# architector1324/micro-raytracer

Measured on AMD Instinct MI355X. Metric: Msamples/sec (res x spp), higher is better.
Workload: dtype f32

## Files before the change

### micro_raytracer_amd/csrc/mrt_math.h

```cpp
#pragma once

#include <stdint.h>

#if defined(__HIPCC__) || defined(__HIP__)
#define MRT_HD __host__ __device__ inline __attribute__((always_inline))
#define MRT_HD_NOINLINE __host__ __device__
#else
#define MRT_HD inline __attribute__((always_inline))
#define MRT_HD_NOINLINE
#endif

namespace mrt {

typedef uint32_t u32;
typedef int32_t i32;

MRT_HD u32 f2u(float f) { return __builtin_bit_cast(u32, f); }
MRT_HD float u2f(u32 u) { return __builtin_bit_cast(float, u); }
MRT_HD float fabs_(float x) { return __builtin_fabsf(x); }
MRT_HD float floor_(float x) { return __builtin_floorf(x); }
MRT_HD float trunc_(float x) { return __builtin_truncf(x); }

#if defined(__HIP_DEVICE_COMPILE__) && !defined(MRT_GENERIC_IEEE)
#define MRT_FAST_IEEE 1
MRT_HD bool wave_all(bool ok) { return __builtin_amdgcn_ballot_w64(!ok) == 0ull; }
#else
MRT_HD bool wave_all(bool ok) { return ok; }
#endif
constexpr float kWinLo = 0x1p-40f, kWinHi = 0x1p+40f;
MRT_HD bool in_window(float x) { const float a = fabs_(x); return a >= kWinLo && a <= kWinHi; }
MRT_HD bool in_window_pos(float x) { return x >= kWinLo && x <= kWinHi; }

#if defined(MRT_FAST_IEEE)
MRT_HD float sqrt_core_(float x)
{
    const float s = __builtin_amdgcn_sqrtf(x);
    const float sd = u2f(f2u(s) - 1u), su = u2f(f2u(s) + 1u);
    const float vd = __builtin_fmaf(-sd, s, x), vu = __builtin_fmaf(-su, s, x);
    float r = (0.0f >= vd) ? sd : s;
    r = (0.0f < vu) ? su : r;
    return r;
}
MRT_HD float rcp_refined_(float d)
{
    const float r0 = __builtin_amdgcn_rcpf(d);
    const float e = __builtin_fmaf(-d, r0, 1.0f);
    return __builtin_fmaf(e, r0, r0);
}
MRT_HD float div_core_(float n, float d, float r)
{
    const float q0 = n * r;
    const float q1 = __builtin_fmaf(__builtin_fmaf(-d, q0, n), r, q0);
    return __builtin_fmaf(__builtin_fmaf(-d, q1, n), r, q1);
}
#endif

MRT_HD float sqrt_(float x)
{
#if defined(MRT_FAST_IEEE)
    if (wave_all(in_window_pos(x))) return sqrt_core_(x);
#endif
    return __builtin_sqrtf(x);
}
MRT_HD float recip_(float x)
{
#if defined(MRT_FAST_IEEE)
    if (wave_all(in_window(x))) return div_core_(1.0f, x, rcp_refined_(x));
#endif
    return 1.0f / x;
}
MRT_HD float div_(float a, float b)
{
#if defined(MRT_FAST_IEEE)
    if (wave_all(in_window(a) && in_window(b))) return div_core_(a, b, rcp_refined_(b));
#endif
    return a / b;
}
MRT_HD void div2_(float a0, float a1, float b, float &q0, float &q1)
{
#if defined(MRT_FAST_IEEE)
    if (wave_all(in_window(a0) && in_window(a1) && in_window(b))) {
        const float r = rcp_refined_(b);
        q0 = div_core_(a0, b, r);
        q1 = div_core_(a1, b, r);
        return;
    }
#endif
    q0 = a0 / b;
    q1 = a1 / b;
}
MRT_HD float recip_sqrt_(float m)
{
#if defined(MRT_FAST_IEEE)
    if (wave_all(in_window_pos(m))) {
        const float s = sqrt_core_(m);
        return div_core_(1.0f, s, rcp_refined_(s));
    }
#endif
    return 1.0f / __builtin_sqrtf(m);
}
MRT_HD float rcp_fast(float x)
{
#if defined(__HIP_DEVICE_COMPILE__)
    return __builtin_amdgcn_rcpf(x);
#else
    return 1.0f / x;
#endif
}
MRT_HD float fma_(float a, float b, float c) { return __builtin_fmaf(a, b, c); }
MRT_HD float fma_fast(float a, float b, float c)
{
#if defined(__HIP_DEVICE_COMPILE__)
    return __builtin_fmaf(a, b, c);
#else
    return a * b + c;
#endif
}

constexpr float kPi = 3.14159274101257324f;
constexpr float kPiO2 = 1.57079637050628662f;
constexpr float kPiO4 = 0.785398185253143311f;
constexpr float kInf = __builtin_huge_valf();

MRT_HD float qnan() { return u2f(0x7fc00000u); }

#if defined(__HIP_DEVICE_COMPILE__)
MRT_HD float fmax_(float a, float b) { return __builtin_fmaxf(a, b); }
MRT_HD float fmin_(float a, float b) { return __builtin_fminf(a, b); }
#else
MRT_HD float fmax_(float a, float b)
{
    if (a != a) return b;
    if (b != b) return a;
    if (a == b) return (f2u(a) & 0x80000000u) ? b : a;
    return a < b ? b : a;
}
MRT_HD float fmin_(float a, float b)
{
    if (a != a) return b;
    if (b != b) return a;
    if (a == b) return (f2u(a) & 0x80000000u) ? a : b;
    return b < a ? b : a;
}
#endif

MRT_HD void sincos_(float x, float &s, float &c)
{
    if (!(fabs_(x) <= 65536.0f)) { s = qnan(); c = qnan(); return; }
    const float kf = floor_(fma_(x, 0.636619746685028076f, 0.5f));
    float r = fma_(-kf, 1.5703125f, x);
    r = fma_(-kf, 4.83751296997070312e-4f, r);
    r = fma_(-kf, 7.54978995489188216e-8f, r);
    const float z = r * r;
    const float sp = fma_(fma_(fma_(-1.9515295891e-4f, z, 8.3321608736e-3f), z, -1.6666654611e-1f) * z, r, r);
    const float cp = fma_(fma_(fma_(2.443315711809948e-5f, z, -1.388731625493765e-3f), z, 4.166664568298827e-2f) * z, z,
                          fma_(-0.5f, z, 1.0f));
    const int q = (int)kf & 3;
    float ss = (q & 1) ? cp : sp;
    float cc = (q & 1) ? sp : cp;
    if (q & 2) ss = -ss;
    if ((q + 1) & 2) cc = -cc;
    s = ss;
    c = cc;
}

MRT_HD float asin_core_(float a)
{
    const float z = a * a;
    const float p = fma_(fma_(fma_(fma_(4.2163199048e-2f, z, 2.4181311049e-2f), z, 4.5470025998e-2f), z, 7.4953002686e-2f), z, 1.6666752422e-1f);
    return fma_(p * z, a, a);
}

MRT_HD float acos_(float x)
{
    const float ax = fabs_(x);
    const bool big = ax > 0.5f;
    const float s = sqrt_(0.5f * (1.0f - ax));
    const float p = asin_core_(big ? s : x);
    const float two_p = 2.0f * p;
    const float r_big = (x > 0.0f) ? two_p : kPi - two_p;
    return big ? r_big : kPiO2 - p;
}

MRT_HD float atan_pos_(float t)
{
    float y0, x;
    if (t > 2.414213562373095f) { y0 = kPiO2; x = -recip_(t); }
    else if (t > 0.4142135623730950f) { y0 = kPiO4; x = div_(t - 1.0f, t + 1.0f); }
    else { y0 = 0.0f; x = t; }
    const float z = x * x;
    const float p = fma_(fma_(fma_(8.05374449538e-2f, z, -1.38776856032e-1f), z, 1.99777106478e-1f), z, -3.33329491539e-1f);
    return y0 + fma_(p * z, x, x);
}

MRT_HD float atan2_(float y, float x)
{
    if (x != x || y != y) return qnan();
    const float ay = fabs_(y), ax = fabs_(x);
    float a;
    if (ax == 0.0f) {
        if (ay == 0.0f) return 0.0f;
        a = kPiO2;
    } else if (ay == kInf && ax == kInf) {
        a = kPiO4;
    } else {
        a = atan_pos_(div_(ay, ax));
    }
    if (x < 0.0f) a = kPi - a;
    return (y < 0.0f) ? -a : a;
}

MRT_HD float pow_(float xf, float yf)
{
    if (yf == 0.0f) return 1.0f;
    if (xf != xf || yf != yf) return qnan();
    if (xf < 0.0f) return qnan();
    if (xf == 0.0f) return (yf > 0.0f) ? 0.0f : kInf;
    if (xf == kInf) return (yf > 0.0f) ? kInf : 0.0f;
    if (xf == 1.0f) return 1.0f;
    if (yf == kInf) return (xf > 1.0f) ? kInf : 0.0f;
    if (yf == -kInf) return (xf > 1.0f) ? 0.0f : kInf;

    const double x = (double)xf;
    const uint64_t bits = __builtin_bit_cast(uint64_t, x);
    int e = (int)((bits >> 52) & 0x7ff) - 1023;
    double m = __builtin_bit_cast(double, (bits & 0x000fffffffffffffULL) | 0x3ff0000000000000ULL);
    if (m > 1.4142135623730951) { m = m * 0.5; e = e + 1; }
    const double r = (m - 1.0) / (m + 1.0);
    const double r2 = r * r;
    double p = 1.0 / 23.0;
    p = p * r2 + 1.0 / 21.0;
    p = p * r2 + 1.0 / 19.0;
    p = p * r2 + 1.0 / 17.0;
    p = p * r2 + 1.0 / 15.0;
    p = p * r2 + 1.0 / 13.0;
    p = p * r2 + 1.0 / 11.0;
    p = p * r2 + 1.0 / 9.0;
    p = p * r2 + 1.0 / 7.0;
    p = p * r2 + 1.0 / 5.0;
    p = p * r2 + 1.0 / 3.0;
    p = p * r2 + 1.0;
    const double lnm = 2.0 * r * p;
    const double log2x = (double)e + lnm * 1.4426950408889634;
    const double t = (double)yf * log2x;
    if (t >= 129.0) return kInf;
    if (t <= -151.0) return 0.0f;
    const double kf = __builtin_floor(t + 0.5);
    const double f = (t - kf) * 0.6931471805599453;
    double q = 1.0 / 6227020800.0;
    q = q * f + 1.0 / 479001600.0;
    q = q * f + 1.0 / 39916800.0;
    q = q * f + 1.0 / 3628800.0;
    q = q * f + 1.0 / 362880.0;
    q = q * f + 1.0 / 40320.0;
    q = q * f + 1.0 / 5040.0;
    q = q * f + 1.0 / 720.0;
    q = q * f + 1.0 / 120.0;
    q = q * f + 1.0 / 24.0;
    q = q * f + 1.0 / 6.0;
    q = q * f + 0.5;
// ... 39 lines not shown
```

### micro_raytracer_amd/csrc/mrt_trace.h

```cpp
#pragma once
#include "mrt_scene.h"

namespace mrt {

enum : u32 {
    F_BOX = 1u,
    F_TRI = 2u,
    F_MAPS = 4u,
    F_LIGHTS = 8u,
    F_ALL = 15u,
    F_BVH = 16u,
    F_NOSTASH = 32u,
    F_COLD = 64u,
    F_DEEP = 128u,
    F_IDENT = 256u
};
constexpr u32 plain_feat(u32 feat) { return feat & ~(u32)F_IDENT; }
MRT_HD u32 staged_words_for(const Params &P, u32 feat) { return (feat & F_DEEP) ? P.lds_words_hot : ((feat & F_COLD) ? P.lds_words_warm : P.lds_words); }
constexpr bool has_walk_area(u32 feat) { return (feat & F_TRI) && (feat & F_BOX) && (feat & F_COLD); }
#ifndef MRT_UNIFORM_TAG
#define MRT_UNIFORM_TAG 1
#endif
#ifndef MRT_T0_FROM_KEY
#define MRT_T0_FROM_KEY 1
#endif
#ifndef MRT_NZFIN_PRODUCT
#define MRT_NZFIN_PRODUCT 1
#endif
#ifndef MRT_SHADOW_QUEUE
#define MRT_SHADOW_QUEUE 0
#endif
#ifndef MRT_LEAF_QUEUE
#define MRT_LEAF_QUEUE 8u
#endif
constexpr u32 kLeafQueue = MRT_LEAF_QUEUE;

#ifndef MRT_PROBE
#define MRT_PROBE(phase)
#endif
#ifndef MRT_COUNT
#define MRT_COUNT(counter)
#endif
#ifndef MRT_PROBE_INST
#define MRT_PROBE_INST(i)
#endif
#if defined(MRT_PHASE_TIMING) && defined(__HIP_DEVICE_COMPILE__)
#define MRT_TICK(slot) do { const unsigned long long now_ = __builtin_amdgcn_s_memtime(); phase_ticks[slot] += now_ - phase_last; phase_last = now_; } while (0)
#define MRT_TICK_DECL unsigned long long phase_ticks[4] = {0ull, 0ull, 0ull, 0ull}; unsigned long long phase_last = __builtin_amdgcn_s_memtime()
#define MRT_TICK_OUT(dst) do { for (int k_ = 0; k_ < 4; ++k_) (dst)[k_] = phase_ticks[k_]; } while (0)
#else
#define MRT_TICK(slot)
#define MRT_TICK_DECL
#define MRT_TICK_OUT(dst)
#endif
#ifndef MRT_PROBE_FALLBACK
#define MRT_PROBE_FALLBACK(ro, rd, dd)
#endif
#ifndef MRT_PROBE_ROUND
#define MRT_PROBE_ROUND(steps, tris, membs)
#endif
enum : u32 { CT_TRACE = 0, CT_LIN_TEST, CT_BVH_NODE, CT_BVH_TEST, CT_MESH_CALL, CT_MESH_ROOT_HIT, CT_TBVH_NODE, CT_TBVH_TRI, CT_TBVH_TRI_HIT, CT_MEMB_BOX, CT_TRACE_ANY, CT_WALK_OVERFLOW, CT_WALK_ROUND, CT_REF_TRI, CT_REF_BOX, CT_COUNT };
enum : u32 { PH_ITER = 0, PH_REGEN, PH_SPHERE_MATH, PH_PLANE_HIT, PH_SHADE, PH_NORMAL_NONPLANE, PH_SCATTER1, PH_SCATTER2, PH_REFRACT, PH_EMIT_END, PH_LIGHTS, PH_COUNT };

constexpr float kE = 0.0001f;
constexpr float kBig = 1.0f / 0.0001f;

struct V3 { float x, y, z; };
MRT_HD V3 v3(float x, float y, float z) { V3 r; r.x = x; r.y = y; r.z = z; return r; }
MRT_HD V3 add(V3 a, V3 b) { return v3(a.x + b.x, a.y + b.y, a.z + b.z); }
MRT_HD V3 sub(V3 a, V3 b) { return v3(a.x - b.x, a.y - b.y, a.z - b.z); }
MRT_HD float dot(V3 a, V3 b) { return a.x * b.x + a.y * b.y + a.z * b.z; }
MRT_HD V3 muls(V3 a, float s) { return v3(a.x * s, a.y * s, a.z * s); }
MRT_HD V3 neg(V3 a) { return v3(-a.x, -a.y, -a.z); }
MRT_HD V3 hadam(V3 a, V3 b) { return v3(a.x * b.x, a.y * b.y, a.z * b.z); }
MRT_HD V3 cross(V3 a, V3 b) { return v3(a.y * b.z - a.z * b.y, a.z * b.x - a.x * b.z, a.x * b.y - a.y * b.x); }
MRT_HD float mag(V3 a) { return sqrt_(a.x * a.x + a.y * a.y + a.z * a.z); }
MRT_HD V3 norm(V3 a) { return muls(a, recip_sqrt_(a.x * a.x + a.y * a.y + a.z * a.z)); }
MRT_HD V3 reflect(V3 d, V3 n) { return sub(d, muls(n, 2.0f * dot(d, n))); }
MRT_HD V3 m3mul(const float *m, V3 v)
{
    return v3(m[0] * v.x + m[1] * v.y + m[2] * v.z, m[3] * v.x + m[4] * v.y + m[5] * v.z, m[6] * v.x + m[7] * v.y + m[8] * v.z);
}
MRT_HD V3 ld3(const float *F, u32 i) { return v3(F[i], F[i + 1], F[i + 2]); }
struct alignas(16) F4 { float x, y, z, w; };
MRT_HD F4 ld4(const float *F, u32 i) { return *reinterpret_cast<const F4 *>(F + i); }
MRT_HD u32 ldu(const float *F, u32 i) { return f2u(F[i]); }

MRT_HD bool nzfin(float x)
{
#if defined(__HIP_DEVICE_COMPILE__)
    return __builtin_amdgcn_classf(x, 0x198);
#else
    const float a = fabs_(x);
    return a > 0.0f && a < kInf;
#endif
}
MRT_HD bool nzfin3(V3 v) { return nzfin(v.x) && nzfin(v.y) && nzfin(v.z); }
MRT_HD bool nzfin3_product(V3 v) { return MRT_NZFIN_PRODUCT ? nzfin((v.x * v.y) * v.z) : nzfin3(v); }
MRT_HD u32 mul24(u32 a, u32 b)
{
    return (a & 0xffffffu) * (b & 0xffffffu);
}
MRT_HD void sched_fence()
{
#if defined(__HIP_DEVICE_COMPILE__)
    __builtin_amdgcn_sched_barrier(0);
#endif
}
MRT_HD u32 opaque_v(u32 x)
{
#if defined(__HIP_DEVICE_COMPILE__)
    asm volatile("" : "+v"(x));
#endif
    return x;
}
MRT_HD u32 opaque_s(u32 x)
{
#if defined(__HIP_DEVICE_COMPILE__)
    asm volatile("" : "+s"(x));
#endif
    return x;
}
MRT_HD u32 lowest_bit(u32 x) { return (u32)__builtin_ctz(x | 0x80000000u); }

MRT_HD V3 xf_full(const float *X, V3 v) { return m3mul(X + XF_R, m3mul(X + XF_L, v)); }
MRT_HD V3 xf_vec(const float *X, bool ident, V3 v)
{
    if (ident && nzfin3_product(v)) return v;
    return xf_full(X, v);
}

MRT_HD V3 recip_patched(V3 d)
{
    V3 m;
#if defined(MRT_FAST_IEEE)
    if (wave_all(in_window(d.x) && in_window(d.y) && in_window(d.z))) {
        m = v3(div_core_(1.0f, d.x, rcp_refined_(d.x)), div_core_(1.0f, d.y, rcp_refined_(d.y)), div_core_(1.0f, d.z, rcp_refined_(d.z)));
        return m;
    }
#endif
    m = v3(1.0f / d.x, 1.0f / d.y, 1.0f / d.z);
    if (fabs_(m.x) == kInf) m.x = kBig;
    if (fabs_(m.y) == kInf) m.y = kBig;
    if (fabs_(m.z) == kInf) m.z = kBig;
    return m;
}

MRT_HD bool box_isect(V3 half, V3 ro, V3 m, V3 pos, float &t0, float &t1)
{
    const V3 n = hadam(sub(ro, pos), m);
    const V3 k = hadam(half, v3(fabs_(m.x), fabs_(m.y), fabs_(m.z)));
    const V3 a = sub(neg(n), k);
    const V3 b = add(neg(n), k);
    t0 = fmax_(fmax_(a.x, a.y), a.z);
    t1 = fmin_(fmin_(b.x, b.y), b.z);
    return !(t0 > t1 || t1 < 0.0f);
}

MRT_HD bool sphere_isect(float r2, V3 oo, V3 rd, float a, float &t0, float &t1)
{
    const float b = 2.0f * dot(oo, rd);
    const float c = dot(oo, oo) - r2;
    const float disc = b * b - 4.0f * a * c;
    if (disc < 0.0f) return false;
    if (b > 1e-20f && a > 0.0f && a < 1e18f && disc >= 0.0f) return false;
    MRT_PROBE(PH_SPHERE_MATH);
    const float sq = sqrt_(disc);
    float q0, q1;
    div2_(-b - sq, -b + sq, 2.0f * a, q0, q1);
    if (q0 < 0.0f) return false;
    t0 = q0;
    t1 = q1;
    return true;
}

MRT_HD bool tri_isect(V3 vp, V3 e0, V3 e1, V3 ro, V3 rd, float &t)
{
    const V3 p = cross(rd, e1);
    const float d = dot(e0, p);
    if (d < kE && d > -kE) return false;
    const float inv_d = recip_(d);
    const V3 tv = sub(ro, vp);
    const float u = dot(tv, p) * inv_d;
    if (u < 0.0f || u > 1.0f) return false;
    const V3 q = cross(tv, e0);
    const float v = dot(rd, q) * inv_d;
    if (v < 0.0f || (u + v) > 1.0f) return false;
    const float tt = dot(e1, q) * inv_d;
    if (tt < 0.0f) return false;
    t = tt;
    return true;
}

MRT_HD bool plane_isect(V3 nn, float d, V3 ro, V3 rd, float &t)
{
    const float tt = div_(-(dot(ro, nn) + d), dot(rd, nn));
    if (tt <= 0.0f) return false;
    t = tt;
    return true;
}

MRT_HD bool in_range(float lo, float hi, float x) { return lo <= x && x < hi; }

MRT_HD V3 box_normal(V3 inv2, V3 hit, V3 pos)
{
    const V3 p = hadam(sub(hit, pos), inv2);
    const float plo = 1.0f - kE, phi = 1.0f + kE, nlo = -1.0f - kE, nhi = -1.0f + kE;
    V3 n = v3(0.0f, 0.0f, 0.0f);
    if (in_range(plo, phi, p.x)) n = v3(1.0f, 0.0f, 0.0f);
    else if (in_range(nlo, nhi, p.x)) n = v3(-1.0f, -0.0f, -0.0f);
    else if (in_range(plo, phi, p.y)) n = v3(0.0f, 1.0f, 0.0f);
    else if (in_range(nlo, nhi, p.y)) n = v3(-0.0f, -1.0f, -0.0f);
    if (in_range(plo, phi, p.z)) n = v3(0.0f, 0.0f, 1.0f);
    else if (in_range(nlo, nhi, p.z)) n = v3(-0.0f, -0.0f, -1.0f);
    return n;
}

struct UV { float x, y; };

MRT_HD UV box_uv(V3 inv2, V3 hit, V3 pos)
{
    const V3 p = hadam(sub(hit, pos), inv2);
    const float plo = 1.0f - kE, phi = 1.0f + kE, nlo = -1.0f - kE, nhi = -1.0f + kE;
    UV r;
    if (in_range(plo, phi, p.x)) { r.x = (0.5f + 0.5f * p.y) / 4.0f + 2.0f / 4.0f; r.y = div_(0.5f - 0.5f * p.z, 3.0f) + 1.0f / 3.0f; }
    else if (in_range(nlo, nhi, p.x)) { r.x = (0.5f - 0.5f * p.y) / 4.0f; r.y = div_(0.5f - 0.5f * p.z, 3.0f) + 1.0f / 3.0f; }
    else if (in_range(plo, phi, p.y)) { r.x = (0.5f - 0.5f * p.x) / 4.0f + 3.0f / 4.0f; r.y = div_(0.5f - 0.5f * p.z, 3.0f) + 1.0f / 3.0f; }
    else if (in_range(nlo, nhi, p.y)) { r.x = (0.5f + 0.5f * p.x) / 4.0f + 1.0f / 4.0f; r.y = div_(0.5f - 0.5f * p.z, 3.0f) + 1.0f / 3.0f; }
    else if (in_range(plo, phi, p.z)) { r.x = (0.5f + 0.5f * p.x) / 4.0f + 1.0f / 4.0f; r.y = div_(0.5f - 0.5f * p.y, 3.0f); }
    else if (in_range(nlo, nhi, p.z)) { r.x = (0.5f + 0.5f * p.x) / 4.0f + 1.0f / 4.0f; r.y = div_(0.5f + 0.5f * p.y, 3.0f) + 2.0f / 3.0f; }
    else { r.x = 0.0f; r.y = 0.0f; }
    return r;
}

MRT_HD float fract_(float x) { return x - trunc_(x); }

MRT_HD uint64_t to_index(float v)
{
    if (!(v > 0.0f)) return 0;
    if (v >= 2147483648.0f) return 2147483648ull;
    return (uint64_t)(u32)v;
}

#if defined(__HIPCC__) || defined(__HIP__)
typedef __attribute__((address_space(3))) volatile float lds_vfloat;
typedef __attribute__((address_space(3))) volatile char lds_char;
#endif

struct Scn {
    const float *F;
    const float *U;
    const float *G;
    const Params *P;
    void *wk;
    u32 wk_stride;
};

struct WalkMem {
#if defined(__HIP_DEVICE_COMPILE__)
    lds_vfloat *b;
    u32 stride;
    MRT_HD explicit WalkMem(const Scn &S) : b((lds_vfloat *)S.wk), stride(S.wk_stride) {}
    MRT_HD void put(u32 e, u32 v) { b[e * stride] = u2f(v); }
    MRT_HD u32 get(u32 e) const { return f2u(b[e * stride]); }
    MRT_HD u32 pitch() const { return stride * 4u; }
    MRT_HD void put_at(u32 off, u32 v) { *(lds_vfloat *)((lds_char *)b + off) = u2f(v); }
#else
    u32 v[kWalkCapMax];
    MRT_HD explicit WalkMem(const Scn &) {}
    MRT_HD void put(u32 e, u32 x) { v[e] = x; }
    MRT_HD u32 get(u32 e) const { return v[e]; }
    MRT_HD u32 pitch() const { return 4u; }
    MRT_HD void put_at(u32 off, u32 x) { v[off >> 2] = x; }
#endif
};

template <u32 FEAT>
MRT_HD V3 tex_fetch(const Scn &S, i32 id, UV uv)
{
    const float *T = S.F + S.P->off_tex + (u32)id * TEX_WORDS;
    const float *X = (FEAT & F_COLD) ? S.G : S.F;
    const u32 w = ldu(T, TEX_W), h = ldu(T, TEX_H), fmt = ldu(T, TEX_FMT), off = ldu(T, TEX_OFF);
    if (fmt == TEXFMT_NONE) return v3(0.0f, 0.0f, 0.0f);
    const uint64_t x = to_index(uv.x * (float)w);
    const uint64_t y = to_index(uv.y * (float)h);
    uint64_t idx = x + y * (uint64_t)w;
    const uint64_t last = (uint64_t)w * h - 1;
    if (idx > last) idx = last;
    const u32 i = (u32)idx;
    if (fmt == TEXFMT_U8) {
        const unsigned char *B = reinterpret_cast<const unsigned char *>(X) + off + i * 3u;
        const float *L = S.F + S.P->off_lut;
        return v3(L[B[0]], L[B[1]], L[B[2]]);
    }
    return ld3(X, off + i * 3u);
}

struct Hit {
    i32 rend;
    u32 inst;
    float t0, t1;
    i32 i0, i1;
};

struct RayPre {
    V3 o, d;
    V3 m;
    float dd;
    bool d_ok;
};

template <u32 FEAT>
MRT_HD RayPre ray_pre(V3 o, V3 d)
{
    RayPre r;
    r.o = o; r.d = d;
    if constexpr (FEAT & F_BOX) r.m = recip_patched(d);
    else r.m = v3(0.0f, 0.0f, 0.0f);
    r.dd = dot(d, d);
    r.d_ok = nzfin3(d);
    return r;
}

struct CullRay {
    V3 o, inv, ainv;
};
MRT_HD float clamp_inv(float d) { return fmin_(fmax_(rcp_fast(d), -1e30f), 1e30f); }
MRT_HD CullRay cull_ray(V3 o, V3 d)
{
    CullRay c;
    c.o = o;
    c.inv = v3(clamp_inv(d.x), clamp_inv(d.y), clamp_inv(d.z));
    c.ainv = v3(fabs_(c.inv.x), fabs_(c.inv.y), fabs_(c.inv.z));
    return c;
}
MRT_HD bool cull_ok(V3 o, float dd)
{
    return nzfin(dd) && dd > 0.98f && dd < 1.02f && fabs_(o.x) < 1e6f && fabs_(o.y) < 1e6f && fabs_(o.z) < 1e6f;
}
#ifndef MRT_MARGIN_SCALE
#define MRT_MARGIN_SCALE 1.0f
#endif
constexpr float kMarginTri = 5e-5f * MRT_MARGIN_SCALE, kMarginPosTri = 1e-6f * MRT_MARGIN_SCALE;
MRT_HD float cull_margin(float k, float kpos, V3 r, V3 h, float big)
{
    const float ext = fmax_(fmax_(fabs_(r.x) + h.x, fabs_(r.y) + h.y), fabs_(r.z) + h.z);
    return fma_fast(k, ext, fma_fast(kpos, big, 1e-6f * MRT_MARGIN_SCALE));
}
MRT_HD bool cull_slab(const CullRay &R, V3 r, V3 h, float mg, float &tn)
// ... 246 lines not shown
        MRT_COUNT(CT_MESH_ROOT_HIT);
        const float *B0 = F + P.off_tbvh;
        const CullRay R = cull_ray(ol, rd);
        V3 oinv, qm;
        {
            const V3 c = ld3(M, MESH_BC), hh = ld3(M, MESH_BH);
            const float big = fmax_(fmax_(fabs_(pos.x), fabs_(pos.y)), fabs_(pos.z)) + fmax_(fmax_(fabs_(c.x) + hh.x, fabs_(c.y) + hh.y), fabs_(c.z) + hh.z)
                              + fmax_(fmax_(fabs_(ol.x), fabs_(ol.y)), fabs_(ol.z));
            const float mg = cull_margin(kMarginTri, kMarginPosTri, sub(c, ol), hh, big);
            oinv = hadam(ol, R.inv);
            qm = muls(R.ainv, mg);
        }
        u32 s0 = 0, s1 = 0;
        u32 node = tb;
        if constexpr ((!ANY || MRT_SHADOW_QUEUE) && has_walk_area(FEAT)) {
            const u32 kQ = P.walk_cap;
            WalkMem q(S);
            for (;;) {
                u32 qo = 0u;
                const u32 q_pitch = opaque_s(q.pitch()), q_full = kQ * q_pitch;
                u32 probe_steps = 0; (void)probe_steps;
                bool walking = node != BVH_END;
                while (walking) {
                    ++probe_steps;
                    const F4 na = ld4(B0, node * BVH_WORDS), nb = ld4(B0, node * BVH_WORDS + 4);
                    MRT_COUNT(CT_TBVH_NODE);
                    const u32 skip = f2u(nb.z);
                    const u32 leaf = opaque_v(f2u(nb.w)), child = node + 1u;
                    const float px = fma_fast(na.x, R.inv.x, -oinv.x), py = fma_fast(na.y, R.inv.y, -oinv.y), pz = fma_fast(na.z, R.inv.z, -oinv.z);
                    const float qx = fma_fast(na.w, R.ainv.x, qm.x), qy = fma_fast(nb.x, R.ainv.y, qm.y), qz = fma_fast(nb.y, R.ainv.z, qm.z);
                    const float tn = fmax_(fmax_(px - qx, py - qy), pz - qz);
                    const float tf = fmin_(fmin_(px + qx, py + qy), pz + qz);
                    const bool hit = !(tn > tf || tf < 0.0f);
                    q.put_at(qo, leaf);
                    qo += (hit && leaf != 0u) ? q_pitch : 0u;
                    node = hit ? child : skip;
                    walking = node != BVH_END && qo < q_full;
                }
                const u32 nq = qo / q_pitch;
                if (nq == 0u) { MRT_PROBE_ROUND(probe_steps, 0u, 0u); break; }
                u32 e = 0u, j = 0u, leaf = q.get(0u), probe_tris = 0; (void)probe_tris;
                while (e < nq) {
                    const u32 id = (leaf & 0xffffffu) + j;
                    ++j; ++probe_tris;
                    if (j == (leaf >> 24)) { ++e; j = 0u; if (e < nq) leaf = q.get(e); }
                    const float *T = CT + P.off_tri + (tri0 + id) * TRI_WORDS;
                    float t;
                    MRT_COUNT(CT_TBVH_TRI);
                    if (!tri_isect(add(ld3(T, 0), pos), ld3(T, 3), ld3(T, 6), ro, rd, t)) continue;
                    MRT_COUNT(CT_TBVH_TRI_HIT);
                    const u32 head = ldu(C, P.off_memb + tri0 + id);
                    const u32 e0 = head & 0xffffffu, ne = head >> 24;
                    u32 sl = 0xffffffffu, sh = 0u;
                    bool cand = false;
                    for (u32 k = 0; k < ne; ++k) {
                        const u32 w = ldu(C, P.off_membe + e0 + k);
                        u32 n = root + (w >> MEMB_SLOT_BITS);
                        bool reached = true;
                        while (n != root) {
                            MRT_COUNT(CT_MEMB_BOX);
                            if (!box_isect(ld3(N0, n * NODE_WORDS + NODE_HALF), ro, m, add(pos, ld3(N0, n * NODE_WORDS + NODE_REL)), a0, a1)) { reached = false; break; }
                            n = ldu(F, P.off_parent + n);
                        }
                        if (!reached) continue;
                        if (ANY) return true;
                        const u32 slot = w & MEMB_SLOT_MASK;
                        if (!cand) sl = slot;
                        sh = slot;
                        cand = true;
                    }
                    if (!cand) continue;
                    const i32 k = total_key(t);
                    if (!any) { any = true; t0 = t1 = t; i0 = i1 = (i32)id; k0 = k1 = k; s0 = sl; s1 = sh; continue; }
                    if (k < k0 || (k == k0 && sl < s0)) { k0 = k; s0 = sl; t0 = t; i0 = (i32)id; }
                    if (k > k1 || (k == k1 && sh > s1)) { k1 = k; s1 = sh; t1 = t; i1 = (i32)id; }
                }
                MRT_PROBE_ROUND(probe_steps, probe_tris, 0u);
                if (node == BVH_END) break;
            }
            return any;
        }
        for (;;) {
            u32 leaf_a = 0u, leaf_b = 0u;
            u32 probe_steps = 0, probe_membs = 0; (void)probe_steps; (void)probe_membs;
            bool walking = node != BVH_END;
            while (walking) {
                ++probe_steps;
                const F4 na = ld4(B0, node * BVH_WORDS), nb = ld4(B0, node * BVH_WORDS + 4);
                MRT_COUNT(CT_TBVH_NODE);
                const u32 skip = f2u(nb.z);
                const u32 leaf = f2u(nb.w), child = node + 1u;
                const float px = fma_fast(na.x, R.inv.x, -oinv.x), py = fma_fast(na.y, R.inv.y, -oinv.y), pz = fma_fast(na.z, R.inv.z, -oinv.z);
                const float qx = fma_fast(na.w, R.ainv.x, qm.x), qy = fma_fast(nb.x, R.ainv.y, qm.y), qz = fma_fast(nb.y, R.ainv.z, qm.z);
                const float tn = fmax_(fmax_(px - qx, py - qy), pz - qz);
                const float tf = fmin_(fmin_(px + qx, py + qy), pz + qz);
                const bool hit = !(tn > tf || tf < 0.0f);
                const u32 cand = hit ? leaf : 0u;
                const bool have_a = leaf_a != 0u;
                leaf_b |= have_a ? cand : 0u;
                leaf_a |= have_a ? 0u : cand;
                node = hit ? child : skip;
                walking = node != BVH_END && leaf_b == 0u;
            }
            if (leaf_a == 0u) { MRT_PROBE_ROUND(probe_steps, 0u, 0u); break; }
            const u32 cnt_a = leaf_a >> 24, first_a = leaf_a & 0xffffffu, cnt_b = leaf_b >> 24, first_b = leaf_b & 0xffffffu;
            MRT_PROBE_ROUND(probe_steps, cnt_a + cnt_b, 0u);
            for (u32 j = 0; j < cnt_a + cnt_b; ++j) {
                const u32 id = j < cnt_a ? first_a + j : first_b + (j - cnt_a);
                const float *T = CT + P.off_tri + (tri0 + id) * TRI_WORDS;
                float t;
                MRT_COUNT(CT_TBVH_TRI);
                if (!tri_isect(add(ld3(T, 0), pos), ld3(T, 3), ld3(T, 6), ro, rd, t)) continue;
                MRT_COUNT(CT_TBVH_TRI_HIT);
                const u32 head = ldu(C, P.off_memb + tri0 + id);
                const u32 e0 = head & 0xffffffu, ne = head >> 24;
                u32 sl = 0xffffffffu, sh = 0u;
                bool cand = false;
                for (u32 e = 0; e < ne; ++e) {
                    const u32 w = ldu(C, P.off_membe + e0 + e);
                    u32 n = root + (w >> MEMB_SLOT_BITS);
                    bool reached = true;
                    while (n != root) {
                        MRT_COUNT(CT_MEMB_BOX);
                        if (!box_isect(ld3(N0, n * NODE_WORDS + NODE_HALF), ro, m, add(pos, ld3(N0, n * NODE_WORDS + NODE_REL)), a0, a1)) { reached = false; break; }
                        n = ldu(F, P.off_parent + n);
                    }
                    if (!reached) continue;
                    if (ANY) return true;
                    const u32 slot = w & MEMB_SLOT_MASK;
                    if (!cand) sl = slot;
                    sh = slot;
                    cand = true;
                }
                if (!cand) continue;
                const i32 k = total_key(t);
                if (!any) { any = true; t0 = t1 = t; i0 = i1 = (i32)id; k0 = k1 = k; s0 = sl; s1 = sh; continue; }
                if (k < k0 || (k == k0 && sl < s0)) { k0 = k; s0 = sl; t0 = t; i0 = (i32)id; }
                if (k > k1 || (k == k1 && sh > s1)) { k1 = k; s1 = sh; t1 = t; i1 = (i32)id; }
            }
        }
        return any;
    }

    count_fallback(P, 7);
    MRT_PROBE_FALLBACK(ro, rd, dd);
    return mesh_isect_ref<ANY, FEAT>(S, mesh, ro, rd, m, pos, t0, i0, t1, i1);
}

#if defined(__HIP_DEVICE_COMPILE__)
MRT_HD u32 wave_uniform(u32 v) { return (u32)__builtin_amdgcn_readfirstlane((int)v); }
#else
MRT_HD u32 wave_uniform(u32 v) { return v; }
#endif
template <bool ANY, u32 FEAT, bool UNIFORM = false>
MRT_HD bool isect_instance(const Scn &S, const RayPre &ray, u32 i, const F4 &ia, const F4 &ib, float &t0, float &t1, i32 &i0, i32 &i1, const float *X0 = nullptr)
{
    const float *F = S.U;
    const Params &P = *S.P;
    const V3 pos = v3(ia.x, ia.y, ia.z);
    const u32 tag = (UNIFORM && (FEAT & F_TRI) && MRT_UNIFORM_TAG) ? wave_uniform(f2u(ib.x)) : f2u(ib.x);
    const u32 kind = (UNIFORM && (FEAT & F_IDENT)) ? wave_uniform(tag & TAG_KIND_MASK) : (tag & TAG_KIND_MASK);
    const bool ident = (FEAT & F_IDENT) ? true : (tag & TAG_IDENT) != 0;
    const float *X = (FEAT & F_IDENT) ? X0 : F + P.off_xf + (tag >> TAG_XF_SHIFT);
    const V3 ro = add(pos, xf_vec(X, ident, sub(ray.o, pos)));
    const bool fast_d = (FEAT & F_IDENT) ? true : (ident && ray.d_ok);
    V3 rd = ray.d, m = ray.m;
    float dd = ray.dd;
    if (!fast_d) {
        rd = xf_full(X, ray.d);
        if constexpr (FEAT & F_BOX) m = recip_patched(rd);
        dd = dot(rd, rd);
    }
    t0 = 0.0f; t1 = 0.0f; i0 = -1; i1 = -1;
    if (kind == KIND_SPHERE) return sphere_isect(ia.w, sub(ro, pos), rd, dd, t0, t1);
    if (kind == KIND_PLANE) { const bool h = plane_isect(v3(ib.y, ib.z, ib.w), ia.w, ro, rd, t0); t1 = t0; return h; }
    if ((FEAT & F_BOX) && kind == KIND_BOX) return box_isect(v3(ia.w, ib.y, ib.z), ro, m, pos, t0, t1);
    if (FEAT & F_TRI) {
        const float *R = F + P.off_rend + ldu(F, P.off_instx + i * INSTX_WORDS + INSTX_REND) * REND_WORDS;
        if (kind == KIND_TRIANGLE) {
            const bool h = tri_isect(add(ld3(R, REND_GEO), pos), ld3(R, REND_GEO + 3), ld3(R, REND_GEO + 6), ro, rd, t0);
            t1 = t0;
            return h;
        }
        if ((FEAT & F_BOX) && kind == KIND_MESH) return mesh_isect<ANY, FEAT>(S, ldu(R, REND_GEO), ro, rd, dd, m, pos, t0, i0, t1, i1);
    }
    return false;
}

template <bool V> struct BoolTag { static constexpr bool value = V; };

template <bool ANY, u32 FEAT>
MRT_HD bool trace(const Scn &S, const RayPre &ray_, Hit &best)
{
    const float *F = S.U;
    const Params &P = *S.P;
    i32 best_key = 0x7fffffff;
    best.rend = -1; best.inst = 0; best.t0 = 0.0f; best.t1 = 0.0f; best.i0 = -1; best.i1 = -1;
    const float *I = F + P.off_inst;

    if (ANY) { MRT_COUNT(CT_TRACE_ANY); } else { MRT_COUNT(CT_TRACE); }
    const float *X0 = nullptr;
    RayPre ray_i = ray_;
    if constexpr (FEAT & F_IDENT) {
        X0 = F + P.off_xf + (ldu(I, INST_TAG) >> TAG_XF_SHIFT);
        if (!ray_.d_ok) {
            ray_i.d = xf_full(X0, ray_.d);
            if constexpr (FEAT & F_BOX) ray_i.m = recip_patched(ray_i.d);
            ray_i.dd = dot(ray_i.d, ray_i.d);
        }
    }
    const RayPre &ray = ray_i;
    auto consider = [&](u32 i, const F4 &ia, const F4 &ib, auto in_order, auto uniform) -> bool {
        float t0, t1;
        MRT_COUNT(CT_LIN_TEST);
        MRT_PROBE_INST(i);
        i32 i0, i1;
        if (!isect_instance<ANY, FEAT, decltype(uniform)::value>(S, ray, i, ia, ib, t0, t1, i0, i1, X0)) return false;
        if (ANY) return true;
        const i32 key = total_key(t0);
        const unsigned long long pair = ((unsigned long long)((u32)key ^ 0x80000000u) << 32) | i;
        const unsigned long long best_pair = ((unsigned long long)((u32)best_key ^ 0x80000000u) << 32) | (best.rend < 0 ? 0xffffffffu : best.inst);
        const bool better = decltype(in_order)::value ? key < best_key : pair < best_pair;
        if (better) {
            best_key = key;
            best.rend = 0; best.inst = i; best.t1 = t1; best.i0 = i0; best.i1 = i1;
            if constexpr ((FEAT & F_BVH) != 0 || !MRT_T0_FROM_KEY) best.t0 = t0;
        }
        return false;
    };
    using InOrder = BoolTag<(FEAT & F_BVH) == 0>;
    using AnyOrder = BoolTag<false>;
    using Shared = BoolTag<true>;
    using PerLane = BoolTag<false>;

    const bool bvh = (FEAT & F_BVH) != 0;
    const u32 n = bvh ? P.n_lin : P.n_inst;
    if (!bvh && !(FEAT & F_TRI) && n) {
        u32 j = 0;
        F4 a0 = ld4(I, 0), a1 = ld4(I, 4), b0 = a0, b1 = a1;
        for (;;) {
            if (j + 1u < n) { b0 = ld4(I, (j + 1u) * INST_WORDS); b1 = ld4(I, (j + 1u) * INST_WORDS + 4); }
            if (consider(j, a0, a1, InOrder(), Shared())) return true;
            if (++j >= n) break;
            if (j + 1u < n) { a0 = ld4(I, (j + 1u) * INST_WORDS); a1 = ld4(I, (j + 1u) * INST_WORDS + 4); }
            if (consider(j, b0, b1, InOrder(), Shared())) return true;
            if (++j >= n) break;
        }
    } else if (n) {
        const float *Lst = F + P.off_lin;
        u32 cur = bvh ? ldu(Lst, 0) : 0u;
        F4 qa = ld4(I, cur * INST_WORDS), qb = ld4(I, cur * INST_WORDS + 4);
        for (u32 j = 0; j < n; ++j) {
            const F4 ia = qa, ib = qb;
            const u32 i = cur;
            if (j + 1 < n) {
                cur = bvh ? ldu(Lst, j + 1) : j + 1;
                qa = ld4(I, cur * INST_WORDS); qb = ld4(I, cur * INST_WORDS + 4);
            }
            if (consider(i, ia, ib, InOrder(), Shared())) return true;
        }
    }

    if constexpr (bvh) {
        const bool cull = cull_ok(ray_.o, ray_.dd);
        const CullRay R = cull_ray(ray_.o, ray_.d);
        const float *N0 = F + P.off_bvh;
        u32 node = P.n_bvh_nodes ? 0u : BVH_END;
        V3 oinv, qm;
        float mg;
        {
            const F4 ra = ld4(N0, 0), rb = ld4(N0, 4);
            const V3 r = sub(v3(ra.x, ra.y, ra.z), R.o);
            const float ext = fmax_(fmax_(fabs_(r.x) + ra.w, fabs_(r.y) + rb.x), fabs_(r.z) + rb.y);
            const float obig = fmax_(fmax_(fabs_(ray_.o.x), fabs_(ray_.o.y)), fabs_(ray_.o.z));
            const float ksq = fmin_(P.inst_ksq * ext, 4e-3f) * MRT_MARGIN_SCALE;
            mg = fma_fast(P.inst_k * MRT_MARGIN_SCALE + ksq, ext, fma_fast(P.inst_kpos * MRT_MARGIN_SCALE, obig + obig + ext, 1e-6f * MRT_MARGIN_SCALE));
            oinv = hadam(R.o, R.inv);
            qm = muls(R.ainv, mg);
        }
        for (;;) {
            u32 leaf_a = 0u, leaf_b = 0u;
            bool walking = node != BVH_END;
            const float far = (!ANY && best.rend >= 0 && best.t0 >= 0.0f) ? best.t0 + 1e-3f * best.t0 + mg : kInf;
            while (walking) {
                const F4 na = ld4(N0, node * BVH_WORDS), nb = ld4(N0, node * BVH_WORDS + 4);
                MRT_COUNT(CT_BVH_NODE);
                const u32 skip = f2u(nb.z), leaf = f2u(nb.w);
                const float px = fma_fast(na.x, R.inv.x, -oinv.x), py = fma_fast(na.y, R.inv.y, -oinv.y), pz = fma_fast(na.z, R.inv.z, -oinv.z);
                const float qx = fma_fast(na.w, R.ainv.x, qm.x), qy = fma_fast(nb.x, R.ainv.y, qm.y), qz = fma_fast(nb.y, R.ainv.z, qm.z);
                const float tn = fmax_(fmax_(px - qx, py - qy), pz - qz);
                const float tf = fmin_(fmin_(px + qx, py + qy), pz + qz);
                bool hit_node = !(tn > tf || tf < 0.0f);
                if (!ANY) hit_node = hit_node && !(tn > far);
                hit_node = hit_node || !cull;
                const u32 cand = hit_node ? leaf : 0u;
                const bool have_a = leaf_a != 0u;
                leaf_b |= have_a ? cand : 0u;
                leaf_a |= have_a ? 0u : cand;
                node = (hit_node && leaf == 0u) ? node + 1u : skip;
                walking = node != BVH_END && leaf_b == 0u;
            }
            if (leaf_a == 0u) break;
            const u32 cnt_a = leaf_a >> 24, first_a = leaf_a & 0xffffffu, cnt_b = leaf_b >> 24, first_b = leaf_b & 0xffffffu;
            for (u32 k = 0; k < cnt_a + cnt_b; ++k) {
                const u32 i = ldu(F, P.off_bvhinst + (k < cnt_a ? first_a + k : first_b + (k - cnt_a)));
                if (consider(i, ld4(I, i * INST_WORDS), ld4(I, i * INST_WORDS + 4), AnyOrder(), PerLane())) return true;
            }
        }
    }
    if (best.rend < 0) return false;
    if constexpr ((FEAT & F_BVH) == 0 && MRT_T0_FROM_KEY) {
        const i32 k = best_key;
        best.t0 = u2f((u32)(k ^ (i32)(((u32)(k >> 31)) >> 1)));
    }
    best.rend = (i32)ldu(S.F, P.off_instx + best.inst * INSTX_WORDS + INSTX_REND);
    return true;
}

struct Obj {
    const float *R, *IX, *X;
    V3 pos;
    bool ident;
    u32 kind;
};
MRT_HD Obj obj_of(const Scn &S, const Hit &h)
{
    Obj o;
    const float *I = S.F + S.P->off_inst + h.inst * INST_WORDS;
    const u32 tag = ldu(I, INST_TAG);
    o.R = S.F + S.P->off_rend + (u32)h.rend * REND_WORDS;
    o.IX = S.F + S.P->off_instx + h.inst * INSTX_WORDS;
    o.X = S.F + S.P->off_xf + (tag >> TAG_XF_SHIFT);
    o.pos = ld3(I, INST_POS);
    o.ident = (tag & TAG_IDENT) != 0;
    o.kind = tag & TAG_KIND_MASK;
    return o;
}
MRT_HD V3 to_object(const Obj &o, V3 hp) { return add(o.pos, xf_vec(o.X, o.ident, sub(hp, o.pos))); }

template <u32 FEAT>
MRT_HD V3 hit_normal(const Scn &S, const Obj &o, V3 n_hit, i32 tri_idx)
{
    if (o.kind == KIND_PLANE) return ld3(o.IX, INSTX_PLANE_NW);
    V3 n = v3(0.0f, 0.0f, 0.0f);
    if (o.kind == KIND_SPHERE) n = sub(n_hit, o.pos);
    else if ((FEAT & F_BOX) && o.kind == KIND_BOX) n = box_normal(ld3(o.R, REND_GEO + 3), n_hit, o.pos);
    else if ((FEAT & F_TRI) && o.kind == KIND_TRIANGLE) n = cross(ld3(o.R, REND_GEO + 3), ld3(o.R, REND_GEO + 6));
    else if (FEAT & F_TRI) {
        const float *M = S.F + S.P->off_mesh + ldu(o.R, REND_GEO) * MESH_WORDS;
        const float *T = ((FEAT & F_DEEP) ? S.G : S.F) + S.P->off_tri + (ldu(M, MESH_TRI0) + (u32)tri_idx) * TRI_WORDS;
        n = cross(ld3(T, 3), ld3(T, 6));
    }
    return norm(xf_vec(o.X, o.ident, n));
}

MRT_HD UV hit_uv(const Obj &o, V3 n_hit)
{
    UV r;
    if (o.kind == KIND_SPHERE) {
        const V3 v = norm(sub(n_hit, o.pos));
        r.x = 0.5f + div_(0.5f * atan2_(v.x, -v.y), kPi);
        r.y = 0.5f - 0.5f * v.z;
    } else if (o.kind == KIND_PLANE) {
        r.x = fract_(n_hit.x + 0.5f);
        if (r.x < 0.0f) r.x = 1.0f + r.x;
        r.y = fract_(n_hit.y + 0.5f);
        if (r.y < 0.0f) r.y = 1.0f + r.y;
    } else if (o.kind == KIND_BOX) {
        r = box_uv(ld3(o.R, REND_GEO + 3), n_hit, o.pos);
    } else {
        r.x = 0.0f; r.y = 0.0f;
    }
    return r;
}

struct Surf {
    const float *M;
    bool maps;
    UV uv;
};
template <u32 FEAT>
MRT_HD Surf surf_of(const Scn &S, const Hit &h, const Obj &o, V3 n_hit)
{
    Surf s;
    s.M = S.F + S.P->off_mat + (u32)h.rend * MAT_WORDS;
    s.maps = false;
    s.uv.x = 0.0f; s.uv.y = 0.0f;
    if constexpr (FEAT & F_MAPS) {
        s.maps = (ldu(o.R, REND_FLAGS) & RF_HAS_MAPS) != 0;
        if (s.maps) s.uv = hit_uv(o, n_hit);
    }
    return s;
}
template <u32 FEAT>
MRT_HD float surf_scalar(const Scn &S, const Surf &s, u32 slot, u32 field)
{
    if (s.maps) {
        const i32 id = (i32)ldu(s.M, MAT_MAP + slot);
        if (id >= 0) return tex_fetch<FEAT>(S, id, s.uv).x;
    }
    return s.M[field];
}
template <u32 FEAT>
MRT_HD V3 surf_color(const Scn &S, const Surf &s)
{
    const V3 albedo = ld3(s.M, MAT_ALBEDO);
    if (s.maps) {
        const i32 id = (i32)ldu(s.M, MAT_MAP + MAP_TEX);
        if (id >= 0) return hadam(albedo, tex_fetch<FEAT>(S, id, s.uv));
    }
    return albedo;
}

MRT_HD V3 rand_normal(V3 n, float r, float u1, float u2)
{
    const float phi = u2 * 2.0f * kPi;
    const float cth = 1.0f - 2.0f * u1;
    const float sth = sqrt_((4.0f * u1) * (1.0f - u1));
    float sphi, cphi;
    sincos_(phi, sphi, cphi);
    const V3 v = v3(sth * cphi, sth * sphi, cth);
    return norm(add(n, muls(v, r)));
}

MRT_HD bool refract(V3 d, float eta, V3 n, V3 &out)
{
    const float cosv = dot(neg(n), d);
    const float k = 1.0f - (eta * eta) * (1.0f - cosv * cosv);
    if (k < 0.0f) return false;
    out = add(muls(d, eta), muls(n, cosv * eta + sqrt_(k)));
    return true;
}

MRT_HD V3 pixel_focus(const Params &P, float cx, float cy)
{
    const float uvx = div_(P.aspect * (cx - 0.5f * P.w), P.w);
    const float uvy = div_(cy - 0.5f * P.h, P.h);
    const V3 dir = norm(v3(uvx, P.inv2tan, -uvy));
    const V3 cam = v3(P.cam_pos[0], P.cam_pos[1], P.cam_pos[2]);
    const V3 orig = add(cam, muls(dir, kE));
    return add(orig, muls(dir, P.foc));
}

MRT_HD V3 lens_pos(const Params &P, u32 pk)
{
    const float u1 = u32_to_unit(draw_u32(pk, DIM_LENS_X));
    const float u2 = u32_to_unit(draw_u32(pk, DIM_LENS_Z));
    return v3(P.cam_pos[0] + (u1 - 0.5f) * P.aprt, P.cam_pos[1], P.cam_pos[2] + (u2 - 0.5f) * P.aprt);
}

MRT_HD void camera_ray(const Params &P, const float *camF, V3 focus, u32 pk, V3 &o, V3 &d)
{
    const float u1 = u32_to_unit(draw_u32(pk, DIM_LENS_X));
    const float u2 = u32_to_unit(draw_u32(pk, DIM_LENS_Z));
    const V3 pos = v3(P.cam_pos[0] + (u1 - 0.5f) * P.aprt, P.cam_pos[1], P.cam_pos[2] + (u2 - 0.5f) * P.aprt);
    const V3 new_dir = norm(sub(focus, pos));
    if (P.cam_ident && nzfin3(new_dir)) d = new_dir;
    else d = m3mul(camF + 9, m3mul(camF, new_dir));
    o = add(pos, muls(d, kE));
}

MRT_HD void camera_ray_centre(const Params &P, const float *camF, V3 focus, V3 &o, V3 &d)
{
    const V3 pos = v3(P.cam_pos[0], P.cam_pos[1], P.cam_pos[2]);
    const V3 new_dir = norm(sub(focus, pos));
    if (P.cam_ident && nzfin3(new_dir)) d = new_dir;
// ... 246 lines not shown
```

Baseline: 9306.

## Screen nearest-hit with approximate reciprocal quotients, redo exactly on ambiguity

In the linear non-triangle instance loop, each sphere or plane candidate is now ranked by an approximate quotient (numerator times hardware reciprocal) instead of an exact division. The exact division is done only once, for the winning instance. If any lane sees a non-normal value, or the two best keys lie within a few ulps, the whole wave reruns the loop with exact divisions. This removes per-candidate IEEE division cost, at the price of extra code, register pressure and occasional full re-traversal.

```diff
diff --git a/micro_raytracer_amd/csrc/mrt_math.h b/micro_raytracer_amd/csrc/mrt_math.h
--- a/micro_raytracer_amd/csrc/mrt_math.h
+++ b/micro_raytracer_amd/csrc/mrt_math.h
@@ -106,6 +106,30 @@
 #else
     return 1.0f / x;
 #endif
+}
+constexpr i32 kQuotUlps = 8;
+MRT_HD bool is_normal_(float x)
+{
+#if defined(__HIP_DEVICE_COMPILE__)
+    return __builtin_amdgcn_classf(x, 0x108);
+#else
+    const float a = fabs_(x);
+    return a >= 0x1p-126f && a <= 0x1.fffffep+127f;
+#endif
+}
+MRT_HD float quot_approx(float n, float d, float r)
+{
+#if defined(__HIP_DEVICE_COMPILE__)
+    (void)d;
+    return n * r;
+#else
+    (void)r;
+    return n / d;
+#endif
+}
+MRT_HD bool quot_ranked(float n, float d, float r, float q)
+{
+    return is_normal_(d) && is_normal_(r) && (is_normal_(q) || n == 0.0f);
 }
 MRT_HD float fma_(float a, float b, float c) { return __builtin_fmaf(a, b, c); }
 MRT_HD float fma_fast(float a, float b, float c)
diff --git a/micro_raytracer_amd/csrc/mrt_trace.h b/micro_raytracer_amd/csrc/mrt_trace.h
--- a/micro_raytracer_amd/csrc/mrt_trace.h
+++ b/micro_raytracer_amd/csrc/mrt_trace.h
@@ -24,6 +24,12 @@
 #ifndef MRT_T0_FROM_KEY
 #define MRT_T0_FROM_KEY 1
 #endif
+#ifndef MRT_SCREEN
+#define MRT_SCREEN 1
+#endif
+#ifndef MRT_SCREEN_HOOK
+#define MRT_SCREEN_HOOK(key, q) (key)
+#endif
 #ifndef MRT_NZFIN_PRODUCT
 #define MRT_NZFIN_PRODUCT 1
 #endif
@@ -157,7 +163,7 @@
     return !(t0 > t1 || t1 < 0.0f);
 }
 
-MRT_HD bool sphere_isect(float r2, V3 oo, V3 rd, float a, float &t0, float &t1)
+MRT_HD bool sphere_terms(float r2, V3 oo, V3 rd, float a, float &n0, float &n1)
 {
     const float b = 2.0f * dot(oo, rd);
     const float c = dot(oo, oo) - r2;
@@ -166,8 +172,15 @@
     if (b > 1e-20f && a > 0.0f && a < 1e18f && disc >= 0.0f) return false;
     MRT_PROBE(PH_SPHERE_MATH);
     const float sq = sqrt_(disc);
-    float q0, q1;
-    div2_(-b - sq, -b + sq, 2.0f * a, q0, q1);
+    n0 = -b - sq;
+    n1 = -b + sq;
+    return true;
+}
+MRT_HD bool sphere_isect(float r2, V3 oo, V3 rd, float a, float &t0, float &t1)
+{
+    float n0, n1, q0, q1;
+    if (!sphere_terms(r2, oo, rd, a, n0, n1)) return false;
+    div2_(n0, n1, 2.0f * a, q0, q1);
     if (q0 < 0.0f) return false;
     t0 = q0;
     t1 = q1;
@@ -192,9 +205,16 @@
     return true;
 }
 
+MRT_HD void plane_terms(V3 nn, float d, V3 ro, V3 rd, float &num, float &den)
+{
+    num = -(dot(ro, nn) + d);
+    den = dot(rd, nn);
+}
 MRT_HD bool plane_isect(V3 nn, float d, V3 ro, V3 rd, float &t)
 {
-    const float tt = div_(-(dot(ro, nn) + d), dot(rd, nn));
+    float num, den;
+    plane_terms(nn, d, ro, rd, num, den);
+    const float tt = div_(num, den);
     if (tt <= 0.0f) return false;
     t = tt;
     return true;
@@ -747,25 +767,43 @@
 #else
 MRT_HD u32 wave_uniform(u32 v) { return v; }
 #endif
+struct InstRay {
+    u32 kind;
+    V3 pos, ro, rd, m;
+    float dd;
+};
+template <u32 FEAT, bool UNIFORM>
+MRT_HD InstRay inst_ray(const Scn &S, const RayPre &ray, const F4 &ia, const F4 &ib, const float *X0)
+{
+    const float *F = S.U;
+    const Params &P = *S.P;
+    InstRay r;
+    r.pos = v3(ia.x, ia.y, ia.z);
+    const u32 tag = (UNIFORM && (FEAT & F_TRI) && MRT_UNIFORM_TAG) ? wave_uniform(f2u(ib.x)) : f2u(ib.x);
+    r.kind = (UNIFORM && (FEAT & F_IDENT)) ? wave_uniform(tag & TAG_KIND_MASK) : (tag & TAG_KIND_MASK);
+    const bool ident = (FEAT & F_IDENT) ? true : (tag & TAG_IDENT) != 0;
+    const float *X = (FEAT & F_IDENT) ? X0 : F + P.off_xf + (tag >> TAG_XF_SHIFT);
+    r.ro = add(r.pos, xf_vec(X, ident, sub(ray.o, r.pos)));
+    const bool fast_d = (FEAT & F_IDENT) ? true : (ident && ray.d_ok);
+    r.rd = ray.d; r.m = ray.m;
+    r.dd = ray.dd;
+    if (!fast_d) {
+        r.rd = xf_full(X, ray.d);
+        if constexpr (FEAT & F_BOX) r.m = recip_patched(r.rd);
+        r.dd = dot(r.rd, r.rd);
+    }
+    return r;
+}
+
 template <bool ANY, u32 FEAT, bool UNIFORM = false>
 MRT_HD bool isect_instance(const Scn &S, const RayPre &ray, u32 i, const F4 &ia, const F4 &ib, float &t0, float &t1, i32 &i0, i32 &i1, const float *X0 = nullptr)
 {
     const float *F = S.U;
     const Params &P = *S.P;
-    const V3 pos = v3(ia.x, ia.y, ia.z);
-    const u32 tag = (UNIFORM && (FEAT & F_TRI) && MRT_UNIFORM_TAG) ? wave_uniform(f2u(ib.x)) : f2u(ib.x);
-    const u32 kind = (UNIFORM && (FEAT & F_IDENT)) ? wave_uniform(tag & TAG_KIND_MASK) : (tag & TAG_KIND_MASK);
-    const bool ident = (FEAT & F_IDENT) ? true : (tag & TAG_IDENT) != 0;
-    const float *X = (FEAT & F_IDENT) ? X0 : F + P.off_xf + (tag >> TAG_XF_SHIFT);
-    const V3 ro = add(pos, xf_vec(X, ident, sub(ray.o, pos)));
-    const bool fast_d = (FEAT & F_IDENT) ? true : (ident && ray.d_ok);
-    V3 rd = ray.d, m = ray.m;
-    float dd = ray.dd;
-    if (!fast_d) {
-        rd = xf_full(X, ray.d);
-        if constexpr (FEAT & F_BOX) m = recip_patched(rd);
-        dd = dot(rd, rd);
-    }
+    const InstRay r = inst_ray<FEAT, UNIFORM>(S, ray, ia, ib, X0);
+    const u32 kind = r.kind;
+    const V3 pos = r.pos, ro = r.ro, rd = r.rd, m = r.m;
+    const float dd = r.dd;
     t0 = 0.0f; t1 = 0.0f; i0 = -1; i1 = -1;
     if (kind == KIND_SPHERE) return sphere_isect(ia.w, sub(ro, pos), rd, dd, t0, t1);
     if (kind == KIND_PLANE) { const bool h = plane_isect(v3(ib.y, ib.z, ib.w), ia.w, ro, rd, t0); t1 = t0; return h; }
@@ -781,6 +819,9 @@
     }
     return false;
 }
+
+MRT_HD float key_to_float(i32 k) { return u2f((u32)(k ^ (i32)(((u32)(k >> 31)) >> 1))); }
+MRT_HD i32 min_i(i32 a, i32 b) { return a < b ? a : b; }
 
 template <bool V> struct BoolTag { static constexpr bool value = V; };
 
@@ -831,16 +872,90 @@
     const bool bvh = (FEAT & F_BVH) != 0;
     const u32 n = bvh ? P.n_lin : P.n_inst;
     if (!bvh && !(FEAT & F_TRI) && n) {
-        u32 j = 0;
-        F4 a0 = ld4(I, 0), a1 = ld4(I, 4), b0 = a0, b1 = a1;
+        bool exact = MRT_SCREEN == 0;
+        i32 amb;
+        bool bad;
+        float w0, w1, wd;
+        auto lin = [&](u32 i, const F4 &ia, const F4 &ib) -> bool {
+            MRT_COUNT(CT_LIN_TEST);
+            MRT_PROBE_INST(i);
+            const InstRay r = inst_ray<FEAT, true>(S, ray, ia, ib, X0);
+            const bool box = (FEAT & F_BOX) && r.kind == KIND_BOX;
+            float n0, n1, den;
+            if (r.kind == KIND_SPHERE) {
+                if (!sphere_terms(ia.w, sub(r.ro, r.pos), r.rd, r.dd, n0, n1)) return false;
+                den = 2.0f * r.dd;
+            } else if (r.kind == KIND_PLANE) {
+                plane_terms(v3(ib.y, ib.z, ib.w), ia.w, r.ro, r.rd, n0, den);
+                n1 = n0;
+            } else if (box) {
+                if (!box_isect(v3(ia.w, ib.y, ib.z), r.ro, r.m, r.pos, n0, n1)) return false;
+                den = 0.0f;
+            } else {
+                return false;
+            }
+            bool hit, ok = true;
+            i32 key;
+            float q1 = n1;
+            if (!exact) {
+                if (box) {
+                    hit = true;
+                    key = total_key(n0);
+                    ok = n0 == n0;
+                } else {
+                    const float rc = rcp_fast(den);
+                    const float q = quot_approx(n0, den, rc);
+                    ok = quot_ranked(n0, den, rc, q);
+                    hit = r.kind == KIND_PLANE ? q > 0.0f : !(q < 0.0f);
+                    key = MRT_SCREEN_HOOK((i32)(f2u(q) & 0x7fffffffu), q);
+                }
+                bad = bad || !ok;
+            } else {
+                float q0 = n0;
+                if (!box) div2_(n0, n1, den, q0, q1);
+                hit = box || (r.kind == KIND_PLANE ? !(q0 <= 0.0f) : !(q0 < 0.0f));
+                key = total_key(q0);
+            }
+            if (ANY) return hit && ok;
+            if (!hit) return false;
+            const bool better = key < best_key;
+            amb = min_i(amb, better ? best_key : key);
+            if (better) {
+                best_key = key;
+                best.rend = 0; best.inst = i; w0 = n0; w1 = q1; wd = den;
+            }
+            return false;
+        };
         for (;;) {
-            if (j + 1u < n) { b0 = ld4(I, (j + 1u) * INST_WORDS); b1 = ld4(I, (j + 1u) * INST_WORDS + 4); }
-            if (consider(j, a0, a1, InOrder(), Shared())) return true;
-            if (++j >= n) break;
-            if (j + 1u < n) { a0 = ld4(I, (j + 1u) * INST_WORDS); a1 = ld4(I, (j + 1u) * INST_WORDS + 4); }
-            if (consider(j, b0, b1, InOrder(), Shared())) return true;
-            if (++j >= n) break;
-        }
+            amb = 0x7fffffff; bad = false;
+            w0 = 1.0f; w1 = 1.0f; wd = 1.0f;
+            u32 j = 0;
+            F4 a0 = ld4(I, 0), a1 = ld4(I, 4), b0 = a0, b1 = a1;
+            for (;;) {
+                if (j + 1u < n) { b0 = ld4(I, (j + 1u) * INST_WORDS); b1 = ld4(I, (j + 1u) * INST_WORDS + 4); }
+                if (lin(j, a0, a1)) return true;
+                if (++j >= n) break;
+                if (j + 1u < n) { a0 = ld4(I, (j + 1u) * INST_WORDS); a1 = ld4(I, (j + 1u) * INST_WORDS + 4); }
+                if (lin(j, b0, b1)) return true;
+                if (++j >= n) break;
+            }
+            if (exact || wave_all(!bad && (ANY || best.rend < 0 || amb > best_key + 2 * kQuotUlps))) break;
+            exact = true;
+            best_key = 0x7fffffff; best.rend = -1; best.inst = 0;
+        }
+        if (ANY || best.rend < 0) return false;
+        if (exact) {
+            best.t0 = key_to_float(best_key);
+            best.t1 = w1;
+        } else {
+            const bool box = (FEAT & F_BOX) && wd == 0.0f;
+            float q0, q1;
+            div2_(w0, w1, box ? 1.0f : wd, q0, q1);
+            best.t0 = box ? w0 : q0;
+            best.t1 = box ? w1 : q1;
+        }
+        best.rend = (i32)ldu(S.F, P.off_instx + best.inst * INSTX_WORDS + INSTX_REND);
+        return true;
     } else if (n) {
         const float *Lst = F + P.off_lin;
         u32 cur = bvh ? ldu(Lst, 0) : 0u;
@@ -905,8 +1020,7 @@
     }
     if (best.rend < 0) return false;
     if constexpr ((FEAT & F_BVH) == 0 && MRT_T0_FROM_KEY) {
-        const i32 k = best_key;
-        best.t0 = u2f((u32)(k ^ (i32)(((u32)(k >> 31)) >> 1)));
+        best.t0 = key_to_float(best_key);
     }
     best.rend = (i32)ldu(S.F, P.off_instx + best.inst * INSTX_WORDS + INSTX_REND);
     return true;
```

Result: slower. 8416, median of 2 (-9.6%).
